# microsoft/esvit

Hardware: NVIDIA H100
Metric: multi-crop images/sec, Swin-T W7 pretrain step (2 global 224^2 + 8 local 96^2 crops, DDINOLoss V+R, K=65536) (higher is better)
Workload: dtype bf16

## Files before the change

### esvit_b200/csrc/gemm2_wgmma.cu

```cuda
#include <cuda.h>

#include "common.cuh"

namespace hg {

constexpr int BK = 64;
constexpr int FOLD_THREADS = 64;
constexpr int SMEM_LIMIT = 232448;
enum { EPI_BIAS = 0, EPI_GELU = 1, EPI_MUL = 2, EPI_F32 = 3 };

__device__ __forceinline__ uint32_t smem_u32(const void* p) { return (uint32_t)__cvta_generic_to_shared(p); }
__device__ __forceinline__ void mbar_init(uint64_t* bar, uint32_t count) {
  asm volatile("mbarrier.init.shared::cta.b64 [%0], %1;\n" ::"r"(smem_u32(bar)), "r"(count));
}
__device__ __forceinline__ void mbar_expect_tx(uint64_t* bar, uint32_t bytes) {
  asm volatile("mbarrier.arrive.expect_tx.shared::cta.b64 _, [%0], %1;\n" ::"r"(smem_u32(bar)), "r"(bytes) : "memory");
}
__device__ __forceinline__ void mbar_arrive(uint64_t* bar) {
  asm volatile("mbarrier.arrive.shared::cta.b64 _, [%0];\n" ::"r"(smem_u32(bar)) : "memory");
}
__device__ __forceinline__ uint64_t global_ns() {
  uint64_t t;
  asm volatile("mov.u64 %0, %%globaltimer;\n" : "=l"(t));
  return t;
// ... 141 lines not shown
}
__device__ __forceinline__ float gelu_fwd(float x) {
  const float x2 = x * x;
  const float th = tanh_approx(x * fmaf(GELU_B, x2, GELU_A));
  const float hx = 0.5f * x;
  return fmaf(hx, th, hx);
}
__device__ __forceinline__ float gelu_fwd_grad(float x, float& dy) {
  const float x2 = x * x;
  const float th = tanh_approx(x * fmaf(GELU_B, x2, GELU_A));
  const float hx = 0.5f * x;
  const float m = fmaf(th, th, -1.f);
  const float nc = fmaf(-3.f * GELU_B, x2, -GELU_A);
  dy = fmaf(hx * m, nc, fmaf(0.5f, th, 0.5f));
  return fmaf(hx, th, hx);
}
constexpr float QGELU_A = 1.702f;
__device__ __forceinline__ float qgelu_fwd(float x) { return x * __frcp_rn(1.f + __expf(-QGELU_A * x)); }
__device__ __forceinline__ float qgelu_fwd_grad(float x, float& dy) {
  const float s = __frcp_rn(1.f + __expf(-QGELU_A * x));
  dy = s * fmaf(QGELU_A * x, 1.f - s, 1.f);
  return x * s;
}

struct Params {
  const float* bias;
  bf16* out;
  bf16* aux;
  float* colsum;
  float* part;
  int M, N, K;
  int splits;
  int kb_per_split;
};

template <int WG, int BN, int EPI>
struct Cfg {
  static constexpr bool PP = WG == 1;
  static constexpr int NEP = PP ? 2 : 1;
  static constexpr int BM = 64 * WG;
  static constexpr int A_BYTES = BM * BK * 2;
  static constexpr int B_BYTES = BN * BK * 2;
  static constexpr int STAGE_BYTES = A_BYTES + B_BYTES;
  static constexpr int BAR_BYTES = PP ? 512 : 256;
  static constexpr int NCHUNK = BN / 64;
  static constexpr int CHUNK_BYTES = BM * 128;
  static constexpr int EP_WG_BYTES = EPI == EPI_BIAS ? 2 * CHUNK_BYTES
                                   : EPI == EPI_GELU ? 4 * CHUNK_BYTES
                                   : EPI == EPI_MUL  ? NCHUNK * CHUNK_BYTES : 0;
  static constexpr int EP_BYTES = NEP * EP_WG_BYTES;
  static constexpr int CS_BYTES = EPI == EPI_MUL ? 8 * BN * 4 : 0;
  static constexpr int STAGES_RAW = (SMEM_LIMIT - 1024  - BAR_BYTES - EP_BYTES - CS_BYTES) / STAGE_BYTES;
  static constexpr int STAGES = STAGES_RAW > 6 ? 6 : STAGES_RAW;
  static constexpr int SMEM = 1024 + STAGES * STAGE_BYTES + EP_BYTES + CS_BYTES + BAR_BYTES;
  static constexpr int NTHREADS = 384;
  static_assert(STAGES >= (BN == 256 && (WG == 2 || EPI == EPI_MUL) ? 3 : 4), "operand ring too shallow");
  static_assert(SMEM <= SMEM_LIMIT, "shared memory budget");
  static_assert((2 * STAGES + 2 * NEP + 2 * NEP * NCHUNK + 2) * 8 <= BAR_BYTES, "mbarrier area");
};

template <int WG, int BN, int EPI, int AMN, int BMN, bool QUICK = false>
__global__ void __launch_bounds__(384, 1) gemm_kernel(const __grid_constant__ CUtensorMap map_a,
                                                      const __grid_constant__ CUtensorMap map_b,
                                                      const __grid_constant__ CUtensorMap map_o,
                                                      const __grid_constant__ CUtensorMap map_x,
                                                      const Params p) {
  using C = Cfg<WG, BN, EPI>;
  constexpr int STAGES = C::STAGES, BM = C::BM, NCHUNK = C::NCHUNK;
  constexpr bool PP = C::PP;
  extern __shared__ __align__(1024) uint8_t smem_raw[];
  uint8_t* tiles = smem_raw + ((1024u - (smem_u32(smem_raw) & 1023u)) & 1023u);
  uint8_t* ep = tiles + STAGES * C::STAGE_BYTES;
  float* cs_part = reinterpret_cast<float*>(ep + C::EP_BYTES);
  uint64_t* full = reinterpret_cast<uint64_t*>(ep + C::EP_BYTES + C::CS_BYTES);
  uint64_t* empty = full + STAGES;
  uint64_t* cs_full = empty + STAGES;
  uint64_t* cs_empty = cs_full + C::NEP;
  uint64_t* mul_full = cs_empty + C::NEP;
  uint64_t* mul_empty = mul_full + C::NEP * NCHUNK;
  uint64_t* turn = mul_empty + C::NEP * NCHUNK;

  const int wg = threadIdx.x >> 7;
  const int m_tiles = (p.M + BM - 1) / BM, n_tiles = (p.N + BN - 1) / BN;
  const int tiles_mn = m_tiles * n_tiles, num_items = tiles_mn * p.splits;
  const int k_blocks = (p.K + BK - 1) / BK;

  if (threadIdx.x == 0) {
    asm volatile("prefetch.tensormap [%0];\n" ::"l"(&map_a) : "memory");
    asm volatile("prefetch.tensormap [%0];\n" ::"l"(&map_b) : "memory");
    for (int i = 0; i < STAGES; i++) { mbar_init(&full[i], 1); mbar_init(&empty[i], 128 * WG); }
    for (int e = 0; e < C::NEP; e++) { mbar_init(&cs_full[e], 4 * WG); mbar_init(&cs_empty[e], FOLD_THREADS); }
    if constexpr (EPI == EPI_MUL)
      for (int i = 0; i < C::NEP * NCHUNK; i++) { mbar_init(&mul_full[i], 1); mbar_init(&mul_empty[i], WG); }
    if constexpr (PP) { mbar_init(&turn[0], 128); mbar_init(&turn[1], 128); }
    asm volatile("fence.mbarrier_init.release.cluster;\n" ::: "memory");
  }
  __syncthreads();

  if (wg == 2) {
    asm volatile("setmaxnreg.dec.sync.aligned.u32 40;\n" ::: "memory");
    if (threadIdx.x == 256) {
      int stage = 0;
      uint32_t phase = 0;
      int local = 0;
      if constexpr (EPI == EPI_MUL) asm volatile("prefetch.tensormap [%0];\n" ::"l"(&map_x) : "memory");
      for (int item = blockIdx.x; item < num_items; item += gridDim.x, local++) {
        const int tile = item % tiles_mn, split = item / tiles_mn;
        const int m0 = (tile / n_tiles) * BM, n0 = (tile % n_tiles) * BN;
        const int kb0 = split * p.kb_per_split;
        int kb1 = kb0 + p.kb_per_split; kb1 = kb1 < k_blocks ? kb1 : k_blocks;
        const int e = PP ? (local & 1) : 0, use = PP ? local >> 1 : local;
        auto load_mul = [&](int j) {
          mbar_wait(&mul_empty[e * NCHUNK + j], (use & 1) ^ 1);
          const uint32_t dst = smem_u32(ep + e * C::EP_WG_BYTES + j * C::CHUNK_BYTES);
          mbar_expect_tx(&mul_full[e * NCHUNK + j], C::CHUNK_BYTES);
#pragma unroll
          for (int h = 0; h < WG; h++)
            tma_load_2d(dst + h * 8192, &map_x, &mul_full[e * NCHUNK + j], n0 + 64 * j, m0 + 64 * h);
        };
        for (int kb = kb0; kb < kb1; kb++) {
          mbar_wait(&empty[stage], phase ^ 1);
          const uint32_t sa = smem_u32(tiles + stage * C::STAGE_BYTES), sb = sa + C::A_BYTES;
          mbar_expect_tx(&full[stage], C::STAGE_BYTES);
          if (!AMN) {
            tma_load_2d(sa, &map_a, &full[stage], kb * BK, m0);
          } else {
#pragma unroll
            for (int j = 0; j < BM / 64; j++)
              tma_load_2d(sa + j * 8192, &map_a, &full[stage], m0 + j * 64, kb * BK);
          }
          if (!BMN) {
            tma_load_2d(sb, &map_b, &full[stage], kb * BK, n0);
          } else {
#pragma unroll
            for (int j = 0; j < BN / 64; j++)
              tma_load_2d(sb + j * 8192, &map_b, &full[stage], n0 + j * 64, kb * BK);
          }
          if (++stage == STAGES) { stage = 0; phase ^= 1; }
          if constexpr (EPI == EPI_MUL) if (kb - kb0 < NCHUNK) load_mul(kb - kb0);
        }
        if constexpr (EPI == EPI_MUL)
          for (int j = kb1 - kb0; j < NCHUNK; j++) load_mul(j);
      }
    } else if (EPI == EPI_MUL && threadIdx.x >= 256 + 32 && threadIdx.x < 256 + 32 + FOLD_THREADS) {
      const int t = threadIdx.x - 256 - 32;
      float* dst = p.colsum + (long long)blockIdx.x * p.N;
      int local = 0;
      for (int item = blockIdx.x; item < num_items; item += gridDim.x, local++) {
        const int n0 = ((item % tiles_mn) % n_tiles) * BN;
        const int e = PP ? (local & 1) : 0, use = PP ? local >> 1 : local;
        mbar_wait(&cs_full[e], use & 1);
        for (int c = t; c < BN && n0 + c < p.N; c += FOLD_THREADS) {
          float sum = 0.f;
#pragma unroll
          for (int w = 0; w < 4 * WG; w++) sum += cs_part[(4 * e + w) * BN + c];
          atomicAdd(dst + n0 + c, sum);
        }
        mbar_arrive(&cs_empty[e]);
      }
    }
  } else {
    asm volatile("setmaxnreg.inc.sync.aligned.u32 232;\n" ::: "memory");
    const int t = threadIdx.x & 127, warp = t >> 5, lane = t & 31;
    const int row0 = PP ? 0 : 64 * wg;
    const int frag_row = row0 + warp * 16 + (lane >> 2);
    const int frag_col = 2 * (lane & 3);
    const uint32_t rows_off = PP ? 0u : (uint32_t)wg * 8192u;
    const int e = PP ? wg : 0;
    uint8_t* const my_ep = ep + e * C::EP_WG_BYTES;
    constexpr uint32_t KSTEP_A = AMN ? (2048 >> 4) : (32 >> 4), KSTEP_B = BMN ? (2048 >> 4) : (32 >> 4);
    int stage = 0;
    uint32_t phase = 0;
    int local = 0;
    for (int item = blockIdx.x; item < num_items; item += gridDim.x, local++) {
      const int tile = item % tiles_mn, split = item / tiles_mn;
      const int m0 = (tile / n_tiles) * BM, n0 = (tile % n_tiles) * BN;
      const int kb0 = split * p.kb_per_split;
      int kb1 = kb0 + p.kb_per_split; kb1 = kb1 < k_blocks ? kb1 : k_blocks;
      if constexpr (PP) {
        if ((local & 1) != wg) {
          stage += kb1 - kb0;
          while (stage >= STAGES) { stage -= STAGES; phase ^= 1; }
          continue;
        }
        if (local > 0) mbar_wait(&turn[wg], ((local - 1) >> 1) & 1);
      }
      const int use = PP ? local >> 1 : local;
      float acc[BN / 2];
      int prev = -1;
      for (int kb = kb0; kb < kb1; kb++) {
        mbar_wait(&full[stage], phase);
        const uint32_t sa = smem_u32(tiles + stage * C::STAGE_BYTES) + rows_off;
        const uint64_t da = make_smem_desc(sa, AMN), db = make_smem_desc(smem_u32(tiles + stage * C::STAGE_BYTES) + C::A_BYTES, BMN);
        wgmma_fence();
#pragma unroll
        for (int k = 0; k < BK / 16; k++)
          wgmma_tile<BN, AMN, BMN>(acc, da + k * KSTEP_A, db + k * KSTEP_B, (kb > kb0 || k != 0) ? 1u : 0u);
        wgmma_commit();
        wgmma_wait<1>();
        if (prev >= 0) mbar_arrive(&empty[prev]);
        prev = stage;
        if (++stage == STAGES) { stage = 0; phase ^= 1; }
      }
      if constexpr (PP) mbar_arrive(&turn[wg ^ 1]);
      wgmma_wait<0>();
      if (prev >= 0) mbar_arrive(&empty[prev]);

      if constexpr (EPI == EPI_F32) {
#pragma unroll
        for (int i = 0; i < BN / 8; i++) {
          const int col = n0 + i * 8 + frag_col;
          if (col >= p.N) continue;
#pragma unroll
          for (int h = 0; h < 2; h++) {
            const int row = m0 + frag_row + 8 * h;
            if (row >= p.M) continue;
            const long long off = (long long)row * p.N + col;
            *reinterpret_cast<float2*>(p.part + (long long)split * p.M * p.N + off) =
                make_float2(acc[4 * i + 2 * h], acc[4 * i + 2 * h + 1]);
          }
        }
        continue;
      }

      if constexpr (EPI == EPI_MUL) mbar_wait(&cs_empty[e], (use & 1) ^ 1);
      const uint32_t lrow = (uint32_t)(warp * 16 + (lane & 15)) * 128u, lsw = lane & 7, lblk = lane >> 4;
      const bool leader = t == 0;
#pragma unroll
      for (int c = 0; c < NCHUNK; c++) {
        uint32_t buf;
        if constexpr (EPI == EPI_MUL) {
          buf = smem_u32(my_ep + c * C::CHUNK_BYTES) + rows_off;
          mbar_wait(&mul_full[e * NCHUNK + c], use & 1);
        } else {
          buf = smem_u32(my_ep + (c & 1) * (EPI == EPI_GELU ? 2 : 1) * C::CHUNK_BYTES) + rows_off;
        }
#pragma unroll
        for (int jj = 0; jj < 8; jj += 2) {
          const int i = c * 8 + jj;
          const uint32_t addr = buf + lrow + (((jj + lblk) ^ lsw) << 4);
          const float* a0 = acc + 4 * i;
          if constexpr (EPI == EPI_MUL) {
            uint32_t m[4];
            ldmatrix_x4(addr, m[0], m[1], m[2], m[3]);
            uint32_t o[4];
            float cs[2][2] = {{0.f, 0.f}, {0.f, 0.f}};
#pragma unroll
            for (int q = 0; q < 4; q++) {
              const float2 mf = unpack_bf162(m[q]);
              o[q] = pack_bf162(a0[2 * q] * mf.x, a0[2 * q + 1] * mf.y);
              const float2 of = unpack_bf162(o[q]);
              cs[q >> 1][0] += of.x; cs[q >> 1][1] += of.y;
            }
            stmatrix_x4(addr, o[0], o[1], o[2], o[3]);
#pragma unroll
            for (int s = 0; s < 2; s++) {
              float cs0 = cs[s][0], cs1 = cs[s][1];
#pragma unroll
              for (int o2 = 4; o2 < 32; o2 <<= 1) {
                cs0 += __shfl_xor_sync(0xffffffffu, cs0, o2);
                cs1 += __shfl_xor_sync(0xffffffffu, cs1, o2);
              }
              if (lane < 4)
                *reinterpret_cast<float2*>(cs_part + (wg * 4 + warp) * BN + (i + s) * 8 + frag_col) = make_float2(cs0, cs1);
            }
          } else {
            float b[4] = {0.f, 0.f, 0.f, 0.f};
            if (p.bias) {
#pragma unroll
              for (int s = 0; s < 2; s++) {
                const int col = n0 + (i + s) * 8 + frag_col;
                if (col < p.N) {
                  const float2 bb = __ldg(reinterpret_cast<const float2*>(p.bias + col));
                  b[2 * s] = bb.x; b[2 * s + 1] = bb.y;
                }
              }
            }
            uint32_t o[4], d[4];
#pragma unroll
            for (int q = 0; q < 4; q++) {
              const float v0 = a0[2 * q] + b[2 * (q >> 1)], v1 = a0[2 * q + 1] + b[2 * (q >> 1) + 1];
              if constexpr (EPI == EPI_GELU) {
                if (p.aux) {
                  float d0, d1;
                  float y0, y1;
                  if constexpr (QUICK) {
                    y0 = qgelu_fwd_grad(v0, d0); y1 = qgelu_fwd_grad(v1, d1);
                  } else {
                    y0 = gelu_fwd_grad(v0, d0); y1 = gelu_fwd_grad(v1, d1);
                  }
                  o[q] = pack_bf162(y0, y1);
                  d[q] = pack_bf162(d0, d1);
                } else if constexpr (QUICK) {
                  o[q] = pack_bf162(qgelu_fwd(v0), qgelu_fwd(v1));
                } else {
                  o[q] = pack_bf162(gelu_fwd(v0), gelu_fwd(v1));
                }
              } else {
                o[q] = pack_bf162(v0, v1);
              }
            }
            stmatrix_x4(addr, o[0], o[1], o[2], o[3]);
            if constexpr (EPI == EPI_GELU)
              if (p.aux) stmatrix_x4(addr + C::CHUNK_BYTES, d[0], d[1], d[2], d[3]);
          }
        }
        fence_proxy_async();
        if constexpr (EPI != EPI_MUL)
          if (leader) bulk_wait_read<0>();
        named_barrier(1 + wg, 128);
        if (leader) {
          const int gc = n0 + 64 * c, gr = m0 + row0;
          if (gc < p.N && gr < p.M) {
            tma_store_2d(&map_o, buf, gc, gr);
            if constexpr (EPI == EPI_GELU)
              if (p.aux) tma_store_2d(&map_x, buf + C::CHUNK_BYTES, gc, gr);
          }
          bulk_commit();
          if constexpr (EPI == EPI_MUL) {
            if (c > 0) { bulk_wait_read<1>(); mbar_arrive(&mul_empty[e * NCHUNK + c - 1]); }
            if (c == NCHUNK - 1) { bulk_wait_read<0>(); mbar_arrive(&mul_empty[e * NCHUNK + c]); }
          }
        }
      }
      if constexpr (EPI == EPI_MUL) {
        __syncwarp();
        if (lane == 0) mbar_arrive(&cs_full[e]);
      }
    }
    if constexpr (EPI != EPI_F32)
      if (t == 0) bulk_wait_all();
  }
}

template <int C>
struct MlpCfg {
  static constexpr int BM = 128, HB = 64;
  static constexpr int KB = (C + 63) / 64;
  static constexpr int NH = 4 * C / HB;
  static constexpr int X_BYTES = KB * BM * 128;
  static constexpr int W1_BYTES = KB * HB * 128;
  static constexpr int W2_BYTES = C * 128;
  static constexpr int STAGE_BYTES = W1_BYTES + W2_BYTES;
  static constexpr int CHUNK_BYTES = BM * 128;
  static constexpr int EP_BYTES = 2 * CHUNK_BYTES;
  static constexpr int BAR_BYTES = 128;
  static constexpr int STAGES_RAW = (SMEM_LIMIT - 1024 - BAR_BYTES - 2 * X_BYTES - EP_BYTES) / STAGE_BYTES;
  static constexpr int STAGES = STAGES_RAW > 4 ? 4 : STAGES_RAW;
  static constexpr int SMEM = 1024 + 2 * X_BYTES + STAGES * STAGE_BYTES + EP_BYTES + BAR_BYTES;
  static_assert(C % 32 == 0 && C <= 192, "acc2 [64 x C] must fit the consumer registers; C / 8 even");
  static_assert(STAGES >= 2, "weight ring too shallow");
  static_assert(SMEM <= SMEM_LIMIT, "shared memory budget");
  static_assert((2 * STAGES + 4) * 8 <= BAR_BYTES, "mbarrier area");
};
// ... 244 lines not shown
                        void* g, int M, void* stream) {
  return h ? mlp_launch<C, true>(x, w1, b1, w2, b2, y, h, g, M, stream)
           : mlp_launch<C, false>(x, w1, b1, w2, b2, y, h, g, M, stream);
}

__global__ void __launch_bounds__(256) colsum_fold_kernel(const float* __restrict__ ws, int rows, int N, float* __restrict__ colsum) {
  const int n = blockIdx.x * 256 + threadIdx.x;
  if (n >= N) return;
  float s = 0.f;
  for (int r = 0; r < rows; r++) s += ws[(long long)r * N + n];
  colsum[n] += s;
}

__global__ void __launch_bounds__(256) split_fold_kernel(const float* __restrict__ part, int splits, long long n4,
                                                         float* __restrict__ out, int accumulate) {
  const long long i = (long long)blockIdx.x * 256 + threadIdx.x;
  if (i >= n4) return;
  float4 s = accumulate ? reinterpret_cast<const float4*>(out)[i] : make_float4(0.f, 0.f, 0.f, 0.f);
  for (int k = 0; k < splits; k++) {
    const float4 t = reinterpret_cast<const float4*>(part)[(long long)k * n4 + i];
    s.x += t.x; s.y += t.y; s.z += t.z; s.w += t.w;
  }
  reinterpret_cast<float4*>(out)[i] = s;
}

constexpr int MAX_GRID = 160;

struct Call {
  const void* a; const void* b;
  int a_mn, b_mn;
  Params p;
};

template <int WG, int BN, int EPI, int AMN, int BMN, bool QUICK = false>
static int launch_cfg(const Call& c, void* stream, int* rows_out) {
  using C = Cfg<WG, BN, EPI>;
  Params p = c.p;
  CUtensorMap ma, mb;
  if (!(AMN ? make_map(&ma, c.a, p.K, p.M, 64) : make_map(&ma, c.a, p.M, p.K, C::BM))) return ESVIT_ERR_BAD_ARG;
  if (!(BMN ? make_map(&mb, c.b, p.K, p.N, 64) : make_map(&mb, c.b, p.N, p.K, BN))) return ESVIT_ERR_BAD_ARG;
  CUtensorMap mo = {}, mx = {};
  if (EPI != EPI_F32) {
    auto aligned = [](const void* q) { return ((uintptr_t)q & 15u) == 0; };
    if (!p.out || !aligned(p.out) || (p.aux && !aligned(p.aux))) return ESVIT_ERR_BAD_ARG;
    if (!make_map(&mo, p.out, p.M, p.N, 64)) return ESVIT_ERR_BAD_ARG;
    if (p.aux && !make_map(&mx, p.aux, p.M, p.N, 64)) return ESVIT_ERR_BAD_ARG;
  }
  auto kernel = gemm_kernel<WG, BN, EPI, AMN, BMN, QUICK>;
  static bool attr_set = false;
  if (!attr_set) {
    cudaError_t e = cudaFuncSetAttribute(kernel, cudaFuncAttributeMaxDynamicSharedMemorySize, C::SMEM);
    if (e != cudaSuccess) return (int)e;
    attr_set = true;
  }
  const int m_tiles = (p.M + C::BM - 1) / C::BM, n_tiles = (p.N + BN - 1) / BN;
  const long long items = (long long)m_tiles * n_tiles * p.splits;
  int grid = esvit_num_sms();
  if (EPI == EPI_MUL && grid > MAX_GRID) grid = MAX_GRID;
  if ((long long)grid > items) grid = (int)items;
  if (EPI == EPI_MUL) {
    cudaError_t e = cudaMemsetAsync(p.colsum, 0, (size_t)grid * p.N * sizeof(float), (cudaStream_t)stream);
    if (e != cudaSuccess) return (int)e;
  }
  if (rows_out) *rows_out = grid;
  kernel<<<grid, C::NTHREADS, C::SMEM, (cudaStream_t)stream>>>(ma, mb, mo, mx, p);
  return (int)cudaGetLastError();
}

template <int WG, int BN, int EPI>
static int launch_majors(const Call& c, void* stream, int* rows_out) {
  if constexpr (EPI == EPI_F32) {
    if (c.a_mn && c.b_mn) return launch_cfg<WG, BN, EPI, 1, 1>(c, stream, rows_out);
  } else if constexpr (EPI == EPI_MUL) {
    if (!c.a_mn) return c.b_mn ? launch_cfg<WG, BN, EPI, 0, 1>(c, stream, rows_out) : launch_cfg<WG, BN, EPI, 0, 0>(c, stream, rows_out);
  } else {
    if (!c.a_mn) return c.b_mn ? launch_cfg<WG, BN, EPI, 0, 1>(c, stream, rows_out) : launch_cfg<WG, BN, EPI, 0, 0>(c, stream, rows_out);
    return c.b_mn ? launch_cfg<WG, BN, EPI, 1, 1>(c, stream, rows_out) : launch_cfg<WG, BN, EPI, 1, 0>(c, stream, rows_out);
  }
  return ESVIT_ERR_BAD_ARG;
}

template <int EPI>
static int launch_epi(const Call& c, int wg, int bn, void* stream, int* rows_out) {
  if (wg == 2 && bn == 256) return launch_majors<2, 256, EPI>(c, stream, rows_out);
  if (wg == 2 && bn == 128) return launch_majors<2, 128, EPI>(c, stream, rows_out);
  if (wg == 1 && bn == 256) return launch_majors<1, 256, EPI>(c, stream, rows_out);
  if (wg == 1 && bn == 128) return launch_majors<1, 128, EPI>(c, stream, rows_out);
  return ESVIT_ERR_BAD_ARG;
}

static int launch_quick(const Call& c, int wg, int bn, void* stream) {
  if (c.a_mn || c.b_mn) return ESVIT_ERR_BAD_ARG;
  if (wg == 2 && bn == 256) return launch_cfg<2, 256, EPI_GELU, 0, 0, true>(c, stream, nullptr);
  if (wg == 2 && bn == 128) return launch_cfg<2, 128, EPI_GELU, 0, 0, true>(c, stream, nullptr);
  if (wg == 1 && bn == 256) return launch_cfg<1, 256, EPI_GELU, 0, 0, true>(c, stream, nullptr);
  if (wg == 1 && bn == 128) return launch_cfg<1, 128, EPI_GELU, 0, 0, true>(c, stream, nullptr);
  return ESVIT_ERR_BAD_ARG;
}

static int launch(const Call& c, int epi, int wg, int bn, void* stream, int* rows_out = nullptr) {
  switch (epi) {
    case EPI_BIAS: return launch_epi<EPI_BIAS>(c, wg, bn, stream, rows_out);
    case EPI_GELU: return launch_epi<EPI_GELU>(c, wg, bn, stream, rows_out);
    case EPI_MUL: return launch_epi<EPI_MUL>(c, wg, bn, stream, rows_out);
    case EPI_F32: return launch_epi<EPI_F32>(c, wg, bn, stream, rows_out);
  }
  return ESVIT_ERR_BAD_ARG;
}

static bool pads_more(long long n, int wide, int narrow) {
  return (n + wide - 1) / wide * wide > (n + narrow - 1) / narrow * narrow;
}
static void pick_tile(long long M, int N, int K, int tile, bool fit_n, int* wg, int* bn) {
  tile %= 10000;
  if (tile > 0) { *wg = tile / 1000; *bn = tile % 1000; return; }
  const int sms = esvit_num_sms();
  const bool narrow = fit_n && (pads_more(N, 256, 128) || K <= 256);
  const int cand[4][2] = {{2, 256}, {2, 128}, {1, 256}, {1, 128}};
  for (const auto& cd : cand) {
    if (cd[1] == 256 && (N <= 128 || narrow)) continue;
    const long long items = ((M + 64 * cd[0] - 1) / (64 * cd[0])) * ((N + cd[1] - 1) / cd[1]);
    if (items >= sms) { *wg = cd[0]; *bn = cd[1]; return; }
  }
  *wg = 1; *bn = 128;
}
static void pick_tile_wgrad(int Nout, int Kin, int tile, int* wg, int* bn) {
  tile %= 10000;
  if (tile > 0) { *wg = tile / 1000; *bn = tile % 1000; return; }
  *bn = Kin > 128 && !pads_more(Kin, 256, 128) ? 256 : 128;
  *wg = Nout > 64 && !pads_more(Nout, 128, 64) ? 2 : 1;
}

}

ESVIT_API int esvit_gemm_bf16(const void* a, const void* b, const float* bias, void* out, void* pre, long long M, int N,
                              int K, int a_mn, int b_mn, int act, int tile, void* stream) {
  if (M <= 0 || N <= 0 || K <= 0 || (N % 8) || (K % 8) || M > 0x7fffffffLL || (a_mn && (M % 8)) || act < 0 || act > 2)
    return ESVIT_ERR_BAD_ARG;
  hg::Call c;
  c.a = a; c.b = b; c.a_mn = a_mn ? 1 : 0; c.b_mn = b_mn ? 1 : 0;
  c.p.bias = bias; c.p.out = (bf16*)out; c.p.aux = act ? (bf16*)pre : nullptr; c.p.colsum = nullptr; c.p.part = nullptr;
  c.p.M = (int)M; c.p.N = N; c.p.K = K; c.p.splits = 1; c.p.kb_per_split = (K + hg::BK - 1) / hg::BK;
  int wg, bn;
  hg::pick_tile(M, N, K, tile, true, &wg, &bn);
  if (act == 2) return hg::launch_quick(c, wg, bn, stream);
  return hg::launch(c, act ? hg::EPI_GELU : hg::EPI_BIAS, wg, bn, stream);
}

ESVIT_API int esvit_gemm_mul_colsum2(const void* a, const void* b, const void* mult, void* out, float* colsum, float* ws,
                                     long long M, int N, int K, int b_mn, int tile, void* stream) {
  if (M <= 0 || N <= 0 || K <= 0 || (N % 8) || (K % 8) || M > 0x7fffffffLL || !mult || !colsum || !ws) return ESVIT_ERR_BAD_ARG;
  hg::Call c;
  c.a = a; c.b = b; c.a_mn = 0; c.b_mn = b_mn ? 1 : 0;
  c.p.bias = nullptr; c.p.out = (bf16*)out; c.p.aux = (bf16*)mult; c.p.colsum = ws; c.p.part = nullptr;
  c.p.M = (int)M; c.p.N = N; c.p.K = K; c.p.splits = 1; c.p.kb_per_split = (K + hg::BK - 1) / hg::BK;
  int wg, bn, rows = 0;
  hg::pick_tile(M, N, K, tile, false, &wg, &bn);
  const int rc = hg::launch(c, hg::EPI_MUL, wg, bn, stream, &rows);
  if (rc != 0) return rc;
  hg::colsum_fold_kernel<<<(N + 255) / 256, 256, 0, (cudaStream_t)stream>>>(ws, rows, N, colsum);
  ESVIT_LAUNCH_CHECK();
}

static long long wgrad_ws_floats(int N, int K) {
  const int tiles = ((N + 127) / 128) * ((K + 255) / 256);
  long long splits = (2LL * 160 + tiles - 1) / tiles;
  if (splits > 96) splits = 96;
  if (splits < 1) splits = 1;
  return splits * (long long)N * K;
}
ESVIT_API int esvit_gemm_wgrad_ws_floats(int N, int K) {
  const long long n = wgrad_ws_floats(N, K);
  return n > 0x7fffffffLL ? -1 : (int)n;
}
ESVIT_API int esvit_gemm_wgrad(const void* dy, const void* x, float* dw, float* ws, long long T, int N, int K,
                               int accumulate, int tile, void* stream) {
  if (T <= 0 || N <= 0 || K <= 0 || (N % 8) || (K % 8) || T > 0x7fffffffLL || !dw || !ws) return ESVIT_ERR_BAD_ARG;
  auto aligned = [](const void* q) { return ((uintptr_t)q & 15u) == 0; };
  if (!aligned(dw) || !aligned(ws)) return ESVIT_ERR_BAD_ARG;
  int wg, bn;
  hg::pick_tile_wgrad(N, K, tile, &wg, &bn);
  const int m_tiles = (N + 64 * wg - 1) / (64 * wg), n_tiles = (K + bn - 1) / bn;
  const int tiles = m_tiles * n_tiles;
  const int k_blocks = (int)((T + hg::BK - 1) / hg::BK);
  const int ctas = esvit_num_sms();
  int splits = tiles >= ctas ? 1 : ctas / tiles;
  if (splits > k_blocks / 8) splits = k_blocks / 8;
  if (tile >= 10000) splits = tile / 10000;
  const long long cap = wgrad_ws_floats(N, K) / ((long long)N * K);
  if (splits > cap) splits = (int)cap;
  if (splits > k_blocks) splits = k_blocks;
  if (splits < 1) splits = 1;
  int kbs = (k_blocks + splits - 1) / splits;
  splits = (k_blocks + kbs - 1) / kbs;
  hg::Call c;
  c.a = dy; c.b = x; c.a_mn = 1; c.b_mn = 1;
  c.p.bias = nullptr; c.p.out = nullptr; c.p.aux = nullptr; c.p.colsum = nullptr; c.p.part = ws;
  c.p.M = N; c.p.N = K; c.p.K = (int)T; c.p.splits = splits; c.p.kb_per_split = kbs;
  const int rc = hg::launch(c, hg::EPI_F32, wg, bn, stream);
  if (rc != 0) return rc;
  const long long n4 = (long long)N * K / 4;
  hg::split_fold_kernel<<<(unsigned)((n4 + 255) / 256), 256, 0, (cudaStream_t)stream>>>(ws, splits, n4, dw, accumulate);
  ESVIT_LAUNCH_CHECK();
}

ESVIT_API int esvit_mlp_fwd(const void* x, const void* w1, const float* b1, const void* w2, const float* b2, void* y,
                            void* h, void* gelu_grad, long long M, int C, void* stream) {
  auto aligned = [](const void* q, uintptr_t a) { return ((uintptr_t)q & (a - 1)) == 0; };
  if (M <= 0 || M > 0x7fffffffLL || !x || !w1 || !w2 || !y || (h == nullptr) != (gelu_grad == nullptr)) return ESVIT_ERR_BAD_ARG;
  if (!aligned(x, 16) || !aligned(w1, 16) || !aligned(w2, 16) || !aligned(y, 16) || !aligned(h, 16) ||
      !aligned(gelu_grad, 16) || !aligned(b1, 8) || !aligned(b2, 8))
    return ESVIT_ERR_BAD_ARG;
  switch (C) {
    case 96: return hg::mlp_launch_c<96>(x, w1, b1, w2, b2, y, h, gelu_grad, (int)M, stream);
    case 128: return hg::mlp_launch_c<128>(x, w1, b1, w2, b2, y, h, gelu_grad, (int)M, stream);
    case 192: return hg::mlp_launch_c<192>(x, w1, b1, w2, b2, y, h, gelu_grad, (int)M, stream);
  }
  return ESVIT_ERR_BAD_ARG;
}

ESVIT_API int esvit_gemm_bias_act(const void* a, const void* w, const float* bias, void* out, void* pre, long long M,
                                  int N, int K, int act, void* stream) {
  return esvit_gemm_bf16(a, w, bias, out, pre, M, N, K, 0, 0, act, 0, stream);
}
ESVIT_API int esvit_gemm_mul_colsum(const void* a, const void* w, const void* mult, void* out, float* colsum, float* ws,
                                    long long M, int N, int K, void* stream) {
  return esvit_gemm_mul_colsum2(a, w, mult, out, colsum, ws, M, N, K, 0, 0, stream);
}
```

Before: 1364.

## Add ping-pong schedule with 128-row tiles per warpgroup and M-fast tile order

Adds a third GEMM schedule in which each consumer warpgroup owns a full 128-row tile (two 64-row wgmma halves) while the two warpgroups ping-pong across items, and makes it the default first candidate for most shapes. It also adds an m_fast raster option for mapping items to tile origins. The goal is better operand reuse per stage than the 64-row ping-pong, while keeping the epilogue overlap that the cooperative schedule lacks. In exchange it doubles accumulator registers per warpgroup and makes the epilogue more involved.

```diff
diff --git a/esvit_b200/csrc/gemm2_wgmma.cu b/esvit_b200/csrc/gemm2_wgmma.cu
--- a/esvit_b200/csrc/gemm2_wgmma.cu
+++ b/esvit_b200/csrc/gemm2_wgmma.cu
@@ -197,41 +197,55 @@
   int M, N, K;
   int splits;
   int kb_per_split;
+  int m_fast;
 };
 
-template <int WG, int BN, int EPI>
+__device__ __forceinline__ void item_origin(int tile, int m_tiles, int n_tiles, int m_fast, int bm, int bn, int& m0,
+                                            int& n0) {
+  m0 = (m_fast ? tile % m_tiles : tile / n_tiles) * bm;
+  n0 = (m_fast ? tile / m_tiles : tile % n_tiles) * bn;
+}
+
+template <int BM_, bool PP_, int BN, int EPI>
 struct Cfg {
-  static constexpr bool PP = WG == 1;
+  static constexpr int BM = BM_;
+  static constexpr bool PP = PP_;
+  static_assert(BM == 64 || BM == 128, "64- or 128-row items");
+  static_assert(PP || BM == 128, "the cooperative schedule splits a 128-row tile over the two warpgroups");
+  static constexpr int CW = PP ? 1 : 2;
+  static constexpr int MH = BM / 64 / CW;
   static constexpr int NEP = PP ? 2 : 1;
-  static constexpr int BM = 64 * WG;
   static constexpr int A_BYTES = BM * BK * 2;
   static constexpr int B_BYTES = BN * BK * 2;
   static constexpr int STAGE_BYTES = A_BYTES + B_BYTES;
   static constexpr int BAR_BYTES = PP ? 512 : 256;
   static constexpr int NCHUNK = BN / 64;
   static constexpr int CHUNK_BYTES = BM * 128;
-  static constexpr int EP_WG_BYTES = EPI == EPI_BIAS ? 2 * CHUNK_BYTES
-                                   : EPI == EPI_GELU ? 4 * CHUNK_BYTES
+  static constexpr int EBUF_BYTES = (PP ? 64 : BM) * 128;
+  static constexpr int EP_WG_BYTES = EPI == EPI_BIAS ? 2 * EBUF_BYTES
+                                   : EPI == EPI_GELU ? 4 * EBUF_BYTES
                                    : EPI == EPI_MUL  ? NCHUNK * CHUNK_BYTES : 0;
   static constexpr int EP_BYTES = NEP * EP_WG_BYTES;
-  static constexpr int CS_BYTES = EPI == EPI_MUL ? 8 * BN * 4 : 0;
+  static constexpr int CS_ROWS = BM / 16;
+  static constexpr int CS_BYTES = EPI == EPI_MUL ? NEP * CS_ROWS * BN * 4 : 0;
   static constexpr int STAGES_RAW = (SMEM_LIMIT - 1024  - BAR_BYTES - EP_BYTES - CS_BYTES) / STAGE_BYTES;
   static constexpr int STAGES = STAGES_RAW > 6 ? 6 : STAGES_RAW;
   static constexpr int SMEM = 1024 + STAGES * STAGE_BYTES + EP_BYTES + CS_BYTES + BAR_BYTES;
   static constexpr int NTHREADS = 384;
-  static_assert(STAGES >= (BN == 256 && (WG == 2 || EPI == EPI_MUL) ? 3 : 4), "operand ring too shallow");
+  static_assert(STAGES >= (BN == 256 && (BM == 128 || EPI == EPI_MUL) ? 3 : 4), "operand ring too shallow");
   static_assert(SMEM <= SMEM_LIMIT, "shared memory budget");
   static_assert((2 * STAGES + 2 * NEP + 2 * NEP * NCHUNK + 2) * 8 <= BAR_BYTES, "mbarrier area");
+  static_assert(MH * NCHUNK % 2 == 0, "an even number of store steps per item");
 };
 
-template <int WG, int BN, int EPI, int AMN, int BMN, bool QUICK = false>
+template <int BM_, bool PP_, int BN, int EPI, int AMN, int BMN, bool QUICK = false>
 __global__ void __launch_bounds__(384, 1) gemm_kernel(const __grid_constant__ CUtensorMap map_a,
                                                       const __grid_constant__ CUtensorMap map_b,
                                                       const __grid_constant__ CUtensorMap map_o,
                                                       const __grid_constant__ CUtensorMap map_x,
                                                       const Params p) {
-  using C = Cfg<WG, BN, EPI>;
-  constexpr int STAGES = C::STAGES, BM = C::BM, NCHUNK = C::NCHUNK;
+  using C = Cfg<BM_, PP_, BN, EPI>;
+  constexpr int STAGES = C::STAGES, BM = C::BM, NCHUNK = C::NCHUNK, CW = C::CW, MH = C::MH;
   constexpr bool PP = C::PP;
   extern __shared__ __align__(1024) uint8_t smem_raw[];
   uint8_t* tiles = smem_raw + ((1024u - (smem_u32(smem_raw) & 1023u)) & 1023u);
@@ -253,10 +267,10 @@
   if (threadIdx.x == 0) {
     asm volatile("prefetch.tensormap [%0];\n" ::"l"(&map_a) : "memory");
     asm volatile("prefetch.tensormap [%0];\n" ::"l"(&map_b) : "memory");
-    for (int i = 0; i < STAGES; i++) { mbar_init(&full[i], 1); mbar_init(&empty[i], 128 * WG); }
-    for (int e = 0; e < C::NEP; e++) { mbar_init(&cs_full[e], 4 * WG); mbar_init(&cs_empty[e], FOLD_THREADS); }
+    for (int i = 0; i < STAGES; i++) { mbar_init(&full[i], 1); mbar_init(&empty[i], 128 * CW); }
+    for (int e = 0; e < C::NEP; e++) { mbar_init(&cs_full[e], 4 * CW); mbar_init(&cs_empty[e], FOLD_THREADS); }
     if constexpr (EPI == EPI_MUL)
-      for (int i = 0; i < C::NEP * NCHUNK; i++) { mbar_init(&mul_full[i], 1); mbar_init(&mul_empty[i], WG); }
+      for (int i = 0; i < C::NEP * NCHUNK; i++) { mbar_init(&mul_full[i], 1); mbar_init(&mul_empty[i], CW); }
     if constexpr (PP) { mbar_init(&turn[0], 128); mbar_init(&turn[1], 128); }
     asm volatile("fence.mbarrier_init.release.cluster;\n" ::: "memory");
   }
@@ -271,7 +285,8 @@
       if constexpr (EPI == EPI_MUL) asm volatile("prefetch.tensormap [%0];\n" ::"l"(&map_x) : "memory");
       for (int item = blockIdx.x; item < num_items; item += gridDim.x, local++) {
         const int tile = item % tiles_mn, split = item / tiles_mn;
-        const int m0 = (tile / n_tiles) * BM, n0 = (tile % n_tiles) * BN;
+        int m0, n0;
+        item_origin(tile, m_tiles, n_tiles, p.m_fast, BM, BN, m0, n0);
         const int kb0 = split * p.kb_per_split;
         int kb1 = kb0 + p.kb_per_split; kb1 = kb1 < k_blocks ? kb1 : k_blocks;
         const int e = PP ? (local & 1) : 0, use = PP ? local >> 1 : local;
@@ -280,7 +295,7 @@
           const uint32_t dst = smem_u32(ep + e * C::EP_WG_BYTES + j * C::CHUNK_BYTES);
           mbar_expect_tx(&mul_full[e * NCHUNK + j], C::CHUNK_BYTES);
 #pragma unroll
-          for (int h = 0; h < WG; h++)
+          for (int h = 0; h < BM / 64; h++)
             tma_load_2d(dst + h * 8192, &map_x, &mul_full[e * NCHUNK + j], n0 + 64 * j, m0 + 64 * h);
         };
         for (int kb = kb0; kb < kb1; kb++) {
@@ -312,13 +327,14 @@
       float* dst = p.colsum + (long long)blockIdx.x * p.N;
       int local = 0;
       for (int item = blockIdx.x; item < num_items; item += gridDim.x, local++) {
-        const int n0 = ((item % tiles_mn) % n_tiles) * BN;
+        int m0, n0;
+        item_origin(item % tiles_mn, m_tiles, n_tiles, p.m_fast, BM, BN, m0, n0);
         const int e = PP ? (local & 1) : 0, use = PP ? local >> 1 : local;
         mbar_wait(&cs_full[e], use & 1);
         for (int c = t; c < BN && n0 + c < p.N; c += FOLD_THREADS) {
           float sum = 0.f;
 #pragma unroll
-          for (int w = 0; w < 4 * WG; w++) sum += cs_part[(4 * e + w) * BN + c];
+          for (int w = 0; w < C::CS_ROWS; w++) sum += cs_part[(C::CS_ROWS * e + w) * BN + c];
           atomicAdd(dst + n0 + c, sum);
         }
         mbar_arrive(&cs_empty[e]);
@@ -334,12 +350,14 @@
     const int e = PP ? wg : 0;
     uint8_t* const my_ep = ep + e * C::EP_WG_BYTES;
     constexpr uint32_t KSTEP_A = AMN ? (2048 >> 4) : (32 >> 4), KSTEP_B = BMN ? (2048 >> 4) : (32 >> 4);
+    constexpr uint32_t HALF_A = 8192 >> 4;
     int stage = 0;
     uint32_t phase = 0;
     int local = 0;
     for (int item = blockIdx.x; item < num_items; item += gridDim.x, local++) {
       const int tile = item % tiles_mn, split = item / tiles_mn;
-      const int m0 = (tile / n_tiles) * BM, n0 = (tile % n_tiles) * BN;
+      int m0, n0;
+      item_origin(tile, m_tiles, n_tiles, p.m_fast, BM, BN, m0, n0);
       const int kb0 = split * p.kb_per_split;
       int kb1 = kb0 + p.kb_per_split; kb1 = kb1 < k_blocks ? kb1 : k_blocks;
       if constexpr (PP) {
@@ -351,7 +369,7 @@
         if (local > 0) mbar_wait(&turn[wg], ((local - 1) >> 1) & 1);
       }
       const int use = PP ? local >> 1 : local;
-      float acc[BN / 2];
+      float acc[MH][BN / 2];
       int prev = -1;
       for (int kb = kb0; kb < kb1; kb++) {
         mbar_wait(&full[stage], phase);
@@ -360,7 +378,9 @@
         wgmma_fence();
 #pragma unroll
         for (int k = 0; k < BK / 16; k++)
-          wgmma_tile<BN, AMN, BMN>(acc, da + k * KSTEP_A, db + k * KSTEP_B, (kb > kb0 || k != 0) ? 1u : 0u);
+#pragma unroll
+          for (int h = 0; h < MH; h++)
+            wgmma_tile<BN, AMN, BMN>(acc[h], da + h * HALF_A + k * KSTEP_A, db + k * KSTEP_B, (kb > kb0 || k != 0) ? 1u : 0u);
         wgmma_commit();
         wgmma_wait<1>();
         if (prev >= 0) mbar_arrive(&empty[prev]);
@@ -373,16 +393,19 @@
 
       if constexpr (EPI == EPI_F32) {
 #pragma unroll
-        for (int i = 0; i < BN / 8; i++) {
-          const int col = n0 + i * 8 + frag_col;
-          if (col >= p.N) continue;
-#pragma unroll
-          for (int h = 0; h < 2; h++) {
-            const int row = m0 + frag_row + 8 * h;
-            if (row >= p.M) continue;
-            const long long off = (long long)row * p.N + col;
-            *reinterpret_cast<float2*>(p.part + (long long)split * p.M * p.N + off) =
-                make_float2(acc[4 * i + 2 * h], acc[4 * i + 2 * h + 1]);
+        for (int h = 0; h < MH; h++) {
+#pragma unroll
+          for (int i = 0; i < BN / 8; i++) {
+            const int col = n0 + i * 8 + frag_col;
+            if (col >= p.N) continue;
+#pragma unroll
+            for (int r = 0; r < 2; r++) {
+              const int row = m0 + 64 * h + frag_row + 8 * r;
+              if (row >= p.M) continue;
+              const long long off = (long long)row * p.N + col;
+              *reinterpret_cast<float2*>(p.part + (long long)split * p.M * p.N + off) =
+                  make_float2(acc[h][4 * i + 2 * r], acc[h][4 * i + 2 * r + 1]);
+            }
           }
         }
         continue;
@@ -393,98 +416,104 @@
       const bool leader = t == 0;
 #pragma unroll
       for (int c = 0; c < NCHUNK; c++) {
-        uint32_t buf;
-        if constexpr (EPI == EPI_MUL) {
-          buf = smem_u32(my_ep + c * C::CHUNK_BYTES) + rows_off;
-          mbar_wait(&mul_full[e * NCHUNK + c], use & 1);
-        } else {
-          buf = smem_u32(my_ep + (c & 1) * (EPI == EPI_GELU ? 2 : 1) * C::CHUNK_BYTES) + rows_off;
-        }
-#pragma unroll
-        for (int jj = 0; jj < 8; jj += 2) {
-          const int i = c * 8 + jj;
-          const uint32_t addr = buf + lrow + (((jj + lblk) ^ lsw) << 4);
-          const float* a0 = acc + 4 * i;
-          if constexpr (EPI == EPI_MUL) {
-            uint32_t m[4];
-            ldmatrix_x4(addr, m[0], m[1], m[2], m[3]);
-            uint32_t o[4];
-            float cs[2][2] = {{0.f, 0.f}, {0.f, 0.f}};
-#pragma unroll
-            for (int q = 0; q < 4; q++) {
-              const float2 mf = unpack_bf162(m[q]);
-              o[q] = pack_bf162(a0[2 * q] * mf.x, a0[2 * q + 1] * mf.y);
-              const float2 of = unpack_bf162(o[q]);
-              cs[q >> 1][0] += of.x; cs[q >> 1][1] += of.y;
-            }
-            stmatrix_x4(addr, o[0], o[1], o[2], o[3]);
-#pragma unroll
-            for (int s = 0; s < 2; s++) {
-              float cs0 = cs[s][0], cs1 = cs[s][1];
-#pragma unroll
-              for (int o2 = 4; o2 < 32; o2 <<= 1) {
-                cs0 += __shfl_xor_sync(0xffffffffu, cs0, o2);
-                cs1 += __shfl_xor_sync(0xffffffffu, cs1, o2);
+        if constexpr (EPI == EPI_MUL) mbar_wait(&mul_full[e * NCHUNK + c], use & 1);
+#pragma unroll
+        for (int h = 0; h < MH; h++) {
+          const int step = c * MH + h;
+          uint32_t buf;
+          if constexpr (EPI == EPI_MUL)
+            buf = smem_u32(my_ep + c * C::CHUNK_BYTES) + rows_off + h * 8192u;
+          else
+            buf = smem_u32(my_ep + (step & 1) * (EPI == EPI_GELU ? 2 : 1) * C::EBUF_BYTES) + rows_off;
+          const float* const ah = acc[h];
+#pragma unroll
+          for (int jj = 0; jj < 8; jj += 2) {
+            const int i = c * 8 + jj;
+            const uint32_t addr = buf + lrow + (((jj + lblk) ^ lsw) << 4);
+            const float* a0 = ah + 4 * i;
+            if constexpr (EPI == EPI_MUL) {
+              uint32_t m[4];
+              ldmatrix_x4(addr, m[0], m[1], m[2], m[3]);
+              uint32_t o[4];
+              float cs[2][2] = {{0.f, 0.f}, {0.f, 0.f}};
+#pragma unroll
+              for (int q = 0; q < 4; q++) {
+                const float2 mf = unpack_bf162(m[q]);
+                o[q] = pack_bf162(a0[2 * q] * mf.x, a0[2 * q + 1] * mf.y);
+                const float2 of = unpack_bf162(o[q]);
+                cs[q >> 1][0] += of.x; cs[q >> 1][1] += of.y;
               }
-              if (lane < 4)
-                *reinterpret_cast<float2*>(cs_part + (wg * 4 + warp) * BN + (i + s) * 8 + frag_col) = make_float2(cs0, cs1);
-            }
-          } else {
-            float b[4] = {0.f, 0.f, 0.f, 0.f};
-            if (p.bias) {
+              stmatrix_x4(addr, o[0], o[1], o[2], o[3]);
+              float* const cs_row = cs_part + (C::CS_ROWS * e + (row0 + 64 * h) / 16 + warp) * BN;
 #pragma unroll
               for (int s = 0; s < 2; s++) {
-                const int col = n0 + (i + s) * 8 + frag_col;
-                if (col < p.N) {
-                  const float2 bb = __ldg(reinterpret_cast<const float2*>(p.bias + col));
-                  b[2 * s] = bb.x; b[2 * s + 1] = bb.y;
+                float cs0 = cs[s][0], cs1 = cs[s][1];
+#pragma unroll
+                for (int o2 = 4; o2 < 32; o2 <<= 1) {
+                  cs0 += __shfl_xor_sync(0xffffffffu, cs0, o2);
+                  cs1 += __shfl_xor_sync(0xffffffffu, cs1, o2);
+                }
+                if (lane < 4) *reinterpret_cast<float2*>(cs_row + (i + s) * 8 + frag_col) = make_float2(cs0, cs1);
+              }
+            } else {
+              float b[4] = {0.f, 0.f, 0.f, 0.f};
+              if (p.bias) {
+#pragma unroll
+                for (int s = 0; s < 2; s++) {
+                  const int col = n0 + (i + s) * 8 + frag_col;
+                  if (col < p.N) {
+                    const float2 bb = __ldg(reinterpret_cast<const float2*>(p.bias + col));
+                    b[2 * s] = bb.x; b[2 * s + 1] = bb.y;
+                  }
                 }
               }
+              uint32_t o[4], d[4];
+#pragma unroll
+              for (int q = 0; q < 4; q++) {
+                const float v0 = a0[2 * q] + b[2 * (q >> 1)], v1 = a0[2 * q + 1] + b[2 * (q >> 1) + 1];
+                if constexpr (EPI == EPI_GELU) {
+                  if (p.aux) {
+                    float d0, d1;
+                    float y0, y1;
+                    if constexpr (QUICK) {
+                      y0 = qgelu_fwd_grad(v0, d0); y1 = qgelu_fwd_grad(v1, d1);
+                    } else {
+                      y0 = gelu_fwd_grad(v0, d0); y1 = gelu_fwd_grad(v1, d1);
+                    }
+                    o[q] = pack_bf162(y0, y1);
+                    d[q] = pack_bf162(d0, d1);
+                  } else if constexpr (QUICK) {
+                    o[q] = pack_bf162(qgelu_fwd(v0), qgelu_fwd(v1));
+                  } else {
+                    o[q] = pack_bf162(gelu_fwd(v0), gelu_fwd(v1));
+                  }
+                } else {
+                  o[q] = pack_bf162(v0, v1);
+                }
+              }
+              stmatrix_x4(addr, o[0], o[1], o[2], o[3]);
+              if constexpr (EPI == EPI_GELU)
+                if (p.aux) stmatrix_x4(addr + C::EBUF_BYTES, d[0], d[1], d[2], d[3]);
             }
-            uint32_t o[4], d[4];
-#pragma unroll
-            for (int q = 0; q < 4; q++) {
-              const float v0 = a0[2 * q] + b[2 * (q >> 1)], v1 = a0[2 * q + 1] + b[2 * (q >> 1) + 1];
-              if constexpr (EPI == EPI_GELU) {
-                if (p.aux) {
-                  float d0, d1;
-                  float y0, y1;
-                  if constexpr (QUICK) {
-                    y0 = qgelu_fwd_grad(v0, d0); y1 = qgelu_fwd_grad(v1, d1);
-                  } else {
-                    y0 = gelu_fwd_grad(v0, d0); y1 = gelu_fwd_grad(v1, d1);
-                  }
-                  o[q] = pack_bf162(y0, y1);
-                  d[q] = pack_bf162(d0, d1);
-                } else if constexpr (QUICK) {
-                  o[q] = pack_bf162(qgelu_fwd(v0), qgelu_fwd(v1));
-                } else {
-                  o[q] = pack_bf162(gelu_fwd(v0), gelu_fwd(v1));
-                }
-              } else {
-                o[q] = pack_bf162(v0, v1);
+          }
+          fence_proxy_async();
+          if constexpr (EPI != EPI_MUL)
+            if (leader) bulk_wait_read<0>();
+          named_barrier(1 + wg, 128);
+          if (leader) {
+            const int gc = n0 + 64 * c, gr = m0 + row0 + 64 * h;
+            if (gc < p.N && gr < p.M) {
+              tma_store_2d(&map_o, buf, gc, gr);
+              if constexpr (EPI == EPI_GELU)
+                if (p.aux) tma_store_2d(&map_x, buf + C::EBUF_BYTES, gc, gr);
+            }
+            bulk_commit();
+            if constexpr (EPI == EPI_MUL) {
+              if (h == MH - 1) {
+                if (c > 0) { bulk_wait_read<MH>(); mbar_arrive(&mul_empty[e * NCHUNK + c - 1]); }
+                if (c == NCHUNK - 1) { bulk_wait_read<0>(); mbar_arrive(&mul_empty[e * NCHUNK + c]); }
               }
             }
-            stmatrix_x4(addr, o[0], o[1], o[2], o[3]);
-            if constexpr (EPI == EPI_GELU)
-              if (p.aux) stmatrix_x4(addr + C::CHUNK_BYTES, d[0], d[1], d[2], d[3]);
-          }
-        }
-        fence_proxy_async();
-        if constexpr (EPI != EPI_MUL)
-          if (leader) bulk_wait_read<0>();
-        named_barrier(1 + wg, 128);
-        if (leader) {
-          const int gc = n0 + 64 * c, gr = m0 + row0;
-          if (gc < p.N && gr < p.M) {
-            tma_store_2d(&map_o, buf, gc, gr);
-            if constexpr (EPI == EPI_GELU)
-              if (p.aux) tma_store_2d(&map_x, buf + C::CHUNK_BYTES, gc, gr);
-          }
-          bulk_commit();
-          if constexpr (EPI == EPI_MUL) {
-            if (c > 0) { bulk_wait_read<1>(); mbar_arrive(&mul_empty[e * NCHUNK + c - 1]); }
-            if (c == NCHUNK - 1) { bulk_wait_read<0>(); mbar_arrive(&mul_empty[e * NCHUNK + c]); }
           }
         }
       }
@@ -795,9 +824,9 @@
   Params p;
 };
 
-template <int WG, int BN, int EPI, int AMN, int BMN, bool QUICK = false>
+template <int BM, bool PP, int BN, int EPI, int AMN, int BMN, bool QUICK = false>
 static int launch_cfg(const Call& c, void* stream, int* rows_out) {
-  using C = Cfg<WG, BN, EPI>;
+  using C = Cfg<BM, PP, BN, EPI>;
   Params p = c.p;
   CUtensorMap ma, mb;
   if (!(AMN ? make_map(&ma, c.a, p.K, p.M, 64) : make_map(&ma, c.a, p.M, p.K, C::BM))) return ESVIT_ERR_BAD_ARG;
@@ -809,7 +838,7 @@
     if (!make_map(&mo, p.out, p.M, p.N, 64)) return ESVIT_ERR_BAD_ARG;
     if (p.aux && !make_map(&mx, p.aux, p.M, p.N, 64)) return ESVIT_ERR_BAD_ARG;
   }
-  auto kernel = gemm_kernel<WG, BN, EPI, AMN, BMN, QUICK>;
+  auto kernel = gemm_kernel<BM, PP, BN, EPI, AMN, BMN, QUICK>;
   static bool attr_set = false;
   if (!attr_set) {
     cudaError_t e = cudaFuncSetAttribute(kernel, cudaFuncAttributeMaxDynamicSharedMemorySize, C::SMEM);
@@ -818,6 +847,7 @@
   }
   const int m_tiles = (p.M + C::BM - 1) / C::BM, n_tiles = (p.N + BN - 1) / BN;
   const long long items = (long long)m_tiles * n_tiles * p.splits;
+  p.m_fast = (EPI == EPI_BIAS || EPI == EPI_GELU) && n_tiles > m_tiles ? 1 : 0;
   int grid = esvit_num_sms();
   if (EPI == EPI_MUL && grid > MAX_GRID) grid = MAX_GRID;
   if ((long long)grid > items) grid = (int)items;
@@ -830,68 +860,73 @@
   return (int)cudaGetLastError();
 }
 
-template <int WG, int BN, int EPI>
+template <int BM, bool PP, int BN, int EPI>
 static int launch_majors(const Call& c, void* stream, int* rows_out) {
   if constexpr (EPI == EPI_F32) {
-    if (c.a_mn && c.b_mn) return launch_cfg<WG, BN, EPI, 1, 1>(c, stream, rows_out);
+    if (c.a_mn && c.b_mn) return launch_cfg<BM, PP, BN, EPI, 1, 1>(c, stream, rows_out);
   } else if constexpr (EPI == EPI_MUL) {
-    if (!c.a_mn) return c.b_mn ? launch_cfg<WG, BN, EPI, 0, 1>(c, stream, rows_out) : launch_cfg<WG, BN, EPI, 0, 0>(c, stream, rows_out);
+    if (!c.a_mn) return c.b_mn ? launch_cfg<BM, PP, BN, EPI, 0, 1>(c, stream, rows_out) : launch_cfg<BM, PP, BN, EPI, 0, 0>(c, stream, rows_out);
   } else {
-    if (!c.a_mn) return c.b_mn ? launch_cfg<WG, BN, EPI, 0, 1>(c, stream, rows_out) : launch_cfg<WG, BN, EPI, 0, 0>(c, stream, rows_out);
-    return c.b_mn ? launch_cfg<WG, BN, EPI, 1, 1>(c, stream, rows_out) : launch_cfg<WG, BN, EPI, 1, 0>(c, stream, rows_out);
+    if (!c.a_mn) return c.b_mn ? launch_cfg<BM, PP, BN, EPI, 0, 1>(c, stream, rows_out) : launch_cfg<BM, PP, BN, EPI, 0, 0>(c, stream, rows_out);
+    return c.b_mn ? launch_cfg<BM, PP, BN, EPI, 1, 1>(c, stream, rows_out) : launch_cfg<BM, PP, BN, EPI, 1, 0>(c, stream, rows_out);
   }
   return ESVIT_ERR_BAD_ARG;
 }
 
 template <int EPI>
-static int launch_epi(const Call& c, int wg, int bn, void* stream, int* rows_out) {
-  if (wg == 2 && bn == 256) return launch_majors<2, 256, EPI>(c, stream, rows_out);
-  if (wg == 2 && bn == 128) return launch_majors<2, 128, EPI>(c, stream, rows_out);
-  if (wg == 1 && bn == 256) return launch_majors<1, 256, EPI>(c, stream, rows_out);
-  if (wg == 1 && bn == 128) return launch_majors<1, 128, EPI>(c, stream, rows_out);
+static int launch_epi(const Call& c, int sched, int bn, void* stream, int* rows_out) {
+  if (sched == 2 && bn == 256) return launch_majors<128, false, 256, EPI>(c, stream, rows_out);
+  if (sched == 2 && bn == 128) return launch_majors<128, false, 128, EPI>(c, stream, rows_out);
+  if (sched == 1 && bn == 256) return launch_majors<64, true, 256, EPI>(c, stream, rows_out);
+  if (sched == 1 && bn == 128) return launch_majors<64, true, 128, EPI>(c, stream, rows_out);
+  if (sched == 3 && bn == 128) return launch_majors<128, true, 128, EPI>(c, stream, rows_out);
   return ESVIT_ERR_BAD_ARG;
 }
 
-static int launch_quick(const Call& c, int wg, int bn, void* stream) {
+static int launch_quick(const Call& c, int sched, int bn, void* stream) {
   if (c.a_mn || c.b_mn) return ESVIT_ERR_BAD_ARG;
-  if (wg == 2 && bn == 256) return launch_cfg<2, 256, EPI_GELU, 0, 0, true>(c, stream, nullptr);
-  if (wg == 2 && bn == 128) return launch_cfg<2, 128, EPI_GELU, 0, 0, true>(c, stream, nullptr);
-  if (wg == 1 && bn == 256) return launch_cfg<1, 256, EPI_GELU, 0, 0, true>(c, stream, nullptr);
-  if (wg == 1 && bn == 128) return launch_cfg<1, 128, EPI_GELU, 0, 0, true>(c, stream, nullptr);
+  if (sched == 2 && bn == 256) return launch_cfg<128, false, 256, EPI_GELU, 0, 0, true>(c, stream, nullptr);
+  if (sched == 2 && bn == 128) return launch_cfg<128, false, 128, EPI_GELU, 0, 0, true>(c, stream, nullptr);
+  if (sched == 1 && bn == 256) return launch_cfg<64, true, 256, EPI_GELU, 0, 0, true>(c, stream, nullptr);
+  if (sched == 1 && bn == 128) return launch_cfg<64, true, 128, EPI_GELU, 0, 0, true>(c, stream, nullptr);
+  if (sched == 3 && bn == 128) return launch_cfg<128, true, 128, EPI_GELU, 0, 0, true>(c, stream, nullptr);
   return ESVIT_ERR_BAD_ARG;
 }
 
-static int launch(const Call& c, int epi, int wg, int bn, void* stream, int* rows_out = nullptr) {
+static int launch(const Call& c, int epi, int sched, int bn, void* stream, int* rows_out = nullptr) {
   switch (epi) {
-    case EPI_BIAS: return launch_epi<EPI_BIAS>(c, wg, bn, stream, rows_out);
-    case EPI_GELU: return launch_epi<EPI_GELU>(c, wg, bn, stream, rows_out);
-    case EPI_MUL: return launch_epi<EPI_MUL>(c, wg, bn, stream, rows_out);
-    case EPI_F32: return launch_epi<EPI_F32>(c, wg, bn, stream, rows_out);
+    case EPI_BIAS: return launch_epi<EPI_BIAS>(c, sched, bn, stream, rows_out);
+    case EPI_GELU: return launch_epi<EPI_GELU>(c, sched, bn, stream, rows_out);
+    case EPI_MUL: return launch_epi<EPI_MUL>(c, sched, bn, stream, rows_out);
+    case EPI_F32: return launch_epi<EPI_F32>(c, sched, bn, stream, rows_out);
   }
   return ESVIT_ERR_BAD_ARG;
 }
 
+static int tile_rows(int sched) { return sched == 1 ? 64 : 128; }
 static bool pads_more(long long n, int wide, int narrow) {
   return (n + wide - 1) / wide * wide > (n + narrow - 1) / narrow * narrow;
 }
-static void pick_tile(long long M, int N, int K, int tile, bool fit_n, int* wg, int* bn) {
+static void pick_tile(long long M, int N, int K, int tile, bool fit_n, int* sched, int* bn) {
   tile %= 10000;
-  if (tile > 0) { *wg = tile / 1000; *bn = tile % 1000; return; }
+  if (tile > 0) { *sched = tile / 1000; *bn = tile % 1000; return; }
   const int sms = esvit_num_sms();
   const bool narrow = fit_n && (pads_more(N, 256, 128) || K <= 256);
-  const int cand[4][2] = {{2, 256}, {2, 128}, {1, 256}, {1, 128}};
+  const bool wide_first = !fit_n && K < 256;
+  const int cand[4][2] = {{wide_first ? 2 : 3, wide_first ? 256 : 128}, {3, 128}, {1, 256}, {1, 128}};
   for (const auto& cd : cand) {
     if (cd[1] == 256 && (N <= 128 || narrow)) continue;
-    const long long items = ((M + 64 * cd[0] - 1) / (64 * cd[0])) * ((N + cd[1] - 1) / cd[1]);
-    if (items >= sms) { *wg = cd[0]; *bn = cd[1]; return; }
-  }
-  *wg = 1; *bn = 128;
-}
-static void pick_tile_wgrad(int Nout, int Kin, int tile, int* wg, int* bn) {
+    const int rows = tile_rows(cd[0]);
+    const long long items = ((M + rows - 1) / rows) * ((N + cd[1] - 1) / cd[1]);
+    if (items >= sms) { *sched = cd[0]; *bn = cd[1]; return; }
+  }
+  *sched = 1; *bn = 128;
+}
+static void pick_tile_wgrad(int Nout, int Kin, int tile, int* sched, int* bn) {
   tile %= 10000;
-  if (tile > 0) { *wg = tile / 1000; *bn = tile % 1000; return; }
+  if (tile > 0) { *sched = tile / 1000; *bn = tile % 1000; return; }
   *bn = Kin > 128 && !pads_more(Kin, 256, 128) ? 256 : 128;
-  *wg = Nout > 64 && !pads_more(Nout, 128, 64) ? 2 : 1;
+  *sched = Nout > 64 && !pads_more(Nout, 128, 64) ? 2 : 1;
 }
 
 }
@@ -904,10 +939,10 @@
   c.a = a; c.b = b; c.a_mn = a_mn ? 1 : 0; c.b_mn = b_mn ? 1 : 0;
   c.p.bias = bias; c.p.out = (bf16*)out; c.p.aux = act ? (bf16*)pre : nullptr; c.p.colsum = nullptr; c.p.part = nullptr;
   c.p.M = (int)M; c.p.N = N; c.p.K = K; c.p.splits = 1; c.p.kb_per_split = (K + hg::BK - 1) / hg::BK;
-  int wg, bn;
-  hg::pick_tile(M, N, K, tile, true, &wg, &bn);
-  if (act == 2) return hg::launch_quick(c, wg, bn, stream);
-  return hg::launch(c, act ? hg::EPI_GELU : hg::EPI_BIAS, wg, bn, stream);
+  int sched, bn;
+  hg::pick_tile(M, N, K, tile, true, &sched, &bn);
+  if (act == 2) return hg::launch_quick(c, sched, bn, stream);
+  return hg::launch(c, act ? hg::EPI_GELU : hg::EPI_BIAS, sched, bn, stream);
 }
 
 ESVIT_API int esvit_gemm_mul_colsum2(const void* a, const void* b, const void* mult, void* out, float* colsum, float* ws,
@@ -917,9 +952,9 @@
   c.a = a; c.b = b; c.a_mn = 0; c.b_mn = b_mn ? 1 : 0;
   c.p.bias = nullptr; c.p.out = (bf16*)out; c.p.aux = (bf16*)mult; c.p.colsum = ws; c.p.part = nullptr;
   c.p.M = (int)M; c.p.N = N; c.p.K = K; c.p.splits = 1; c.p.kb_per_split = (K + hg::BK - 1) / hg::BK;
-  int wg, bn, rows = 0;
-  hg::pick_tile(M, N, K, tile, false, &wg, &bn);
-  const int rc = hg::launch(c, hg::EPI_MUL, wg, bn, stream, &rows);
+  int sched, bn, rows = 0;
+  hg::pick_tile(M, N, K, tile, false, &sched, &bn);
+  const int rc = hg::launch(c, hg::EPI_MUL, sched, bn, stream, &rows);
   if (rc != 0) return rc;
   hg::colsum_fold_kernel<<<(N + 255) / 256, 256, 0, (cudaStream_t)stream>>>(ws, rows, N, colsum);
   ESVIT_LAUNCH_CHECK();
@@ -941,9 +976,10 @@
   if (T <= 0 || N <= 0 || K <= 0 || (N % 8) || (K % 8) || T > 0x7fffffffLL || !dw || !ws) return ESVIT_ERR_BAD_ARG;
   auto aligned = [](const void* q) { return ((uintptr_t)q & 15u) == 0; };
   if (!aligned(dw) || !aligned(ws)) return ESVIT_ERR_BAD_ARG;
-  int wg, bn;
-  hg::pick_tile_wgrad(N, K, tile, &wg, &bn);
-  const int m_tiles = (N + 64 * wg - 1) / (64 * wg), n_tiles = (K + bn - 1) / bn;
+  int sched, bn;
+  hg::pick_tile_wgrad(N, K, tile, &sched, &bn);
+  const int bm = hg::tile_rows(sched);
+  const int m_tiles = (N + bm - 1) / bm, n_tiles = (K + bn - 1) / bn;
   const int tiles = m_tiles * n_tiles;
   const int k_blocks = (int)((T + hg::BK - 1) / hg::BK);
   const int ctas = esvit_num_sms();
@@ -960,7 +996,7 @@
   c.a = dy; c.b = x; c.a_mn = 1; c.b_mn = 1;
   c.p.bias = nullptr; c.p.out = nullptr; c.p.aux = nullptr; c.p.colsum = nullptr; c.p.part = ws;
   c.p.M = N; c.p.N = K; c.p.K = (int)T; c.p.splits = splits; c.p.kb_per_split = kbs;
-  const int rc = hg::launch(c, hg::EPI_F32, wg, bn, stream);
+  const int rc = hg::launch(c, hg::EPI_F32, sched, bn, stream);
   if (rc != 0) return rc;
   const long long n4 = (long long)N * K / 4;
   hg::split_fold_kernel<<<(unsigned)((n4 + 255) / 256), 256, 0, (cudaStream_t)stream>>>(ws, splits, n4, dw, accumulate);
```

New measurement: 1395, median of 6. 1.02x the previous value.
